# spaceandtimefdn/blitzar

Hardware: NVIDIA H100
Metric: MSM throughput (scalar*point terms/sec), ristretto255, n=2^20 per GPU (higher is better)
Workload: dtype u32 limbs (integer modular arithmetic)

## Files before the change

### blitzar_b200/csrc/curve.cuh

```cuda
#pragma once
#include "field.cuh"

namespace b200 {

enum CurveId : unsigned { kRistretto255 = 0, kBls12381 = 1, kBn254 = 2, kGrumpkin = 3 };

struct SeqExec {
  static constexpr int kLanes = 1;
  template <class F>
  static B200_HD void mul4(typename F::E& o0, typename F::E& o1, typename F::E& o2,
                           typename F::E& o3, const typename F::E& a0, const typename F::E& b0,
                           const typename F::E& a1, const typename F::E& b1,
                           const typename F::E& a2, const typename F::E& b2,
                           const typename F::E& a3, const typename F::E& b3) {
    F::mul(o0, a0, b0);
    F::mul(o1, a1, b1);
    F::mul(o2, a2, b2);
    F::mul(o3, a3, b3);
  }
  template <class F>
  static B200_HD void mul2(typename F::E& o0, typename F::E& o1, const typename F::E& a0,
                           const typename F::E& b0, const typename F::E& a1,
                           const typename F::E& b1) {
    F::mul(o0, a0, b0);
// ... 75 lines not shown
  struct Gen {
    fe YpX, YmX, Z2, T2d;
  };

  static B200_HD Point identity() {
    Point p;
    p.X = F::zero();
    p.Y = F::one();
    p.Z = F::one();
    p.T = F::zero();
    return p;
  }
  static B200_HD void neg(Point& r, const Point& a) {
    F::neg(r.X, a.X);
    r.Y = a.Y;
    r.Z = a.Z;
    F::neg(r.T, a.T);
  }
  template <class X = SeqExec> static B200_HD void add(Point& r, const Point& a, const Point& b) {
    fe A, B, C, D, E, Fv, G, H, t0, t1, t2, t3;
    F::sub(t0, a.Y, a.X);
    F::sub(t1, b.Y, b.X);
    F::add(t2, a.Y, a.X);
    F::add(t3, b.Y, b.X);
    X::template mul4<F>(A, B, C, D, t0, t1, t2, t3, a.T, b.T, a.Z, b.Z);
    F::mul(C, C, F::constant([](int i) { return F25_D2(i); }));
    F::dbl(D, D);
    F::sub(E, B, A);
    F::sub(Fv, D, C);
    F::add(G, D, C);
    F::add(H, B, A);
    Point o;
    X::template mul4<F>(o.X, o.Y, o.T, o.Z, E, Fv, G, H, E, H, Fv, G);
    r = o;
  }
  static B200_HD void point_to_gen(Gen& g, const Point& p) {
    F::add(g.YpX, p.Y, p.X);
    F::sub(g.YmX, p.Y, p.X);
    F::dbl(g.Z2, p.Z);
    F::mul(g.T2d, p.T, F::constant([](int i) { return F25_D2(i); }));
    F::canonical(g.YpX, g.YpX);
    F::canonical(g.YmX, g.YmX);
    F::canonical(g.Z2, g.Z2);
    F::canonical(g.T2d, g.T2d);
  }

  static B200_HD fe denominator(const Point& p) { return p.Z; }
  static B200_HD void normalized_gen(Gen& g, const Point& p, const fe& zi) {
    Point a;
    F::mul(a.X, p.X, zi);
    F::mul(a.Y, p.Y, zi);
    a.Z = F::one();
    F::mul(a.T, a.X, a.Y);
    point_to_gen(g, a);
  }
  static B200_HD void gen_to_point(Point& r, const Gen& g, bool negate) {
    fe x2, t2, nx, nt;
    F::sub(x2, g.YpX, g.YmX);
    F::add(r.Y, g.YpX, g.YmX);
    r.Z = g.Z2;
    F::mul(t2, g.T2d, F::constant([](int i) { return F25_INVD(i); }));
    F::neg(nx, x2);
    F::neg(nt, t2);
    F::select(r.X, x2, nx, negate);
    F::select(r.T, t2, nt, negate);
  }
  template <class X = SeqExec>
  static B200_HD void add_gen(Point& r, const Point& a, const Gen& g, bool negate,
                              bool unit_z = false) {
    fe A, B, C, D, E, Fv, G, H, t0, t1, qp, qm, qt, nt;
    F::select(qp, g.YpX, g.YmX, negate);
    F::select(qm, g.YmX, g.YpX, negate);
    F::neg(nt, g.T2d);
    F::select(qt, g.T2d, nt, negate);
    F::sub(t0, a.Y, a.X);
    F::add(t1, a.Y, a.X);
    if (unit_z) {
      F::mul(A, t0, qm);
      F::mul(B, t1, qp);
      F::mul(C, a.T, qt);
      F::dbl(D, a.Z);
    } else {
      X::template mul4<F>(A, B, C, D, t0, qm, t1, qp, a.T, qt, a.Z, g.Z2);
    }
    F::sub(E, B, A);
    F::sub(Fv, D, C);
    F::add(G, D, C);
    F::add(H, B, A);
    Point o;
    X::template mul4<F>(o.X, o.Y, o.T, o.Z, E, Fv, G, H, E, H, Fv, G);
    r = o;
  }
  template <class X = SeqExec> static B200_HD void dbl(Point& r, const Point& a) {
    fe A, B, C, E, Fv, G, H, t0, t1;
    F::add(t0, a.X, a.Y);
    X::template mul4<F>(A, B, C, t1, a.X, a.X, a.Y, a.Y, a.Z, a.Z, t0, t0);
    F::dbl(C, C);
    F::add(H, A, B);
    F::sub(E, H, t1);
    F::sub(G, A, B);
    F::add(Fv, C, G);
    Point o;
    X::template mul4<F>(o.X, o.Y, o.T, o.Z, E, Fv, G, H, E, H, Fv, G);
    r = o;
  }

  static B200_HD Gen load_unit_gen(const Gen* src) {
    Gen g;
    g.YpX = src->YpX;
    g.YmX = src->YmX;
    g.T2d = src->T2d;
    g.Z2 = F::zero();
    g.Z2.l[0] = 2;
    return g;
  }

  static B200_HD void load_point_abi(Point& p, const void* src) {
    const u64* s = (const u64*)src;
    F::from_radix51(p.X, s);
    F::from_radix51(p.Y, s + 5);
    F::from_radix51(p.Z, s + 10);
    F::from_radix51(p.T, s + 15);
  }
  static B200_HD fe load_abi_z(const void* src) {
    fe z;
    F::from_radix51(z, (const u64*)src + 10);
    return z;
  }
  static B200_HD void load_gen_abi(Gen& g, const void* src) {
    Point p;
    load_point_abi(p, src);
    point_to_gen(g, p);
  }
  static B200_HD void load_proj_abi(Gen& g, const void* src) { load_gen_abi(g, src); }
  static constexpr int kAbiCompactBytes = 120;
  static B200_HD void load_compact_abi(Gen& g, const void* src) {
    const u64* s = (const u64*)src;
    Point p;
    F::from_radix51(p.X, s);
    F::from_radix51(p.Y, s + 5);
    p.Z = F::one();
    F::from_radix51(p.T, s + 10);
    point_to_gen(g, p);
  }
  static B200_HD void store_compact_abi(void* dst, const Point& p, const fe& zi) {
    u64* d = (u64*)dst;
    fe x, y, t;
    F::mul(x, p.X, zi);
    F::mul(y, p.Y, zi);
    F::mul(t, x, y);
    F::to_radix51(d, x);
    F::to_radix51(d + 5, y);
    F::to_radix51(d + 10, t);
  }
  static B200_HD void store_proj_abi(void* dst, const Point& p) {
    u64* d = (u64*)dst;
    F::to_radix51(d, p.X);
    F::to_radix51(d + 5, p.Y);
    F::to_radix51(d + 10, p.Z);
    F::to_radix51(d + 15, p.T);
  }

  struct ScalarPow {
    static B200_HD void pow22523(fe& r, const fe& a) { F::pow22523(r, a); }
  };
  template <class Pow = ScalarPow> static B200_HD int sqrt_ratio_m1(fe& x, const fe& u, const fe& v) {
// ... 182 lines not shown
  }
  static B200_HD bool gen_is_identity(const Gen& g) { return F::is_zero(g.y) && F::is_zero(g.x); }
  static B200_HD Gen subgroup_generator() {
    Gen g;
#pragma unroll
    for (int i = 0; i < N; ++i) {
      g.x.l[i] = F::Params::gx(i);
      g.y.l[i] = F::Params::gy(i);
    }
    return g;
  }
  static B200_HD void neg(Point& r, const Point& a) {
    r.X = a.X;
    F::neg(r.Y, a.Y);
    r.Z = a.Z;
  }
  static B200_HD void mul_by_3b(fe& r, const fe& a) { CP::template mul_by_3b<F>(r, a); }

  template <class X>
  static B200_HD void finish_add(Point& r, const fe& t0, const fe& t1, const fe& t3, const fe& t4,
                                 const fe& y3, const fe& z3) {
    fe x3a, t2a, y3a, t1a, t0a, z3a;
    X::template mul4<F>(x3a, t2a, y3a, t1a, t4, y3, t3, t1, y3, t0, t1, z3);
    X::template mul2<F>(t0a, z3a, t0, t3, z3, t4);
    F::sub(r.X, t2a, x3a);
    F::add(r.Y, t1a, y3a);
    F::add(r.Z, z3a, t0a);
  }
  template <class X = SeqExec> static B200_HD void add(Point& r, const Point& p, const Point& q) {
    fe t0, t1, t2, t3, t4, m3, m4, m5, u0, u1, v0, v1, x3, y3, z3;
    F::add(t3, p.X, p.Y);
    F::add(t4, q.X, q.Y);
    F::add(u0, p.Y, p.Z);
    F::add(u1, q.Y, q.Z);
    F::add(v0, p.X, p.Z);
    F::add(v1, q.X, q.Z);
    X::template mul4<F>(t0, t1, t2, m3, p.X, q.X, p.Y, q.Y, p.Z, q.Z, t3, t4);
    X::template mul2<F>(m4, m5, u0, u1, v0, v1);
    F::add(t4, t0, t1);
    F::sub(t3, m3, t4);
    F::add(x3, t1, t2);
    F::sub(t4, m4, x3);
    F::add(y3, t0, t2);
    F::sub(y3, m5, y3);
    F::add(x3, t0, t0);
    F::add(t0, x3, t0);
    mul_by_3b(t2, t2);
    F::add(z3, t1, t2);
    F::sub(t1, t1, t2);
    mul_by_3b(y3, y3);
    Point o;
    finish_add<X>(o, t0, t1, t3, t4, y3, z3);
    r = o;
  }
  template <class X = SeqExec>
  static B200_HD void add_gen(Point& r, const Point& p, const Gen& g, bool negate,
                              bool  = false) {
    if (gen_is_identity(g)) {
      r = p;
      return;
    }
    fe qy, ny;
    F::neg(ny, g.y);
    F::select(qy, g.y, ny, negate);
    fe t0, t1, t2, t3, t4, m3, x3, y3, z3;
    F::add(t3, g.x, qy);
    F::add(t4, p.X, p.Y);
    X::template mul4<F>(t0, t1, m3, t2, p.X, g.x, p.Y, qy, t3, t4, qy, p.Z);
    F::mul(y3, g.x, p.Z);
    F::add(t4, t0, t1);
    F::sub(t3, m3, t4);
    F::add(t4, t2, p.Y);
    F::add(y3, y3, p.X);
    F::add(x3, t0, t0);
    F::add(t0, x3, t0);
    mul_by_3b(t2, p.Z);
    F::add(z3, t1, t2);
    F::sub(t1, t1, t2);
    mul_by_3b(y3, y3);
    Point o;
    finish_add<X>(o, t0, t1, t3, t4, y3, z3);
    r = o;
  }
  static B200_HD fe denominator(const Point& p) { return F::is_zero(p.Z) ? F::one() : p.Z; }
  static B200_HD void normalized_gen(Gen& g, const Point& p, const fe& zi) {
    if (F::is_zero(p.Z)) {
      g.x = F::zero();
      g.y = F::zero();
      return;
    }
    F::mul(g.x, p.X, zi);
    F::mul(g.y, p.Y, zi);
  }
  static B200_HD void gen_to_point(Point& r, const Gen& g, bool negate) {
    if (gen_is_identity(g)) {
      r = identity();
      return;
    }
    fe ny;
    F::neg(ny, g.y);
    r.X = g.x;
    F::select(r.Y, g.y, ny, negate);
    r.Z = F::one();
  }
  template <class X = SeqExec> static B200_HD void dbl(Point& r, const Point& p) {
    fe t0, t1, t2, txy, x3, y3, z3, xa, xb;
    X::template mul4<F>(t0, t1, t2, txy, p.Y, p.Y, p.Y, p.Z, p.Z, p.Z, p.X, p.Y);
    F::add(z3, t0, t0);
    F::add(z3, z3, z3);
    F::add(z3, z3, z3);
    mul_by_3b(t2, t2);
    F::add(y3, t0, t2);
    fe t22, t23;
    F::add(t22, t2, t2);
    F::add(t23, t22, t2);
    F::sub(t0, t0, t23);
    Point o;
    X::template mul4<F>(xa, o.Z, y3, xb, t2, z3, t1, z3, t0, y3, t0, txy);
    F::add(o.Y, xa, y3);
    F::add(o.X, xb, xb);
    r = o;
  }

  static B200_HD void load_gen_abi(Gen& g, const void* src) {
    const unsigned char* s = (const unsigned char*)src;
    if (s[8 * N]) {
      g.x = F::zero();
      g.y = F::zero();
      return;
    }
    F::load(g.x, s);
    F::load(g.y, s + 4 * N);
  }
  static constexpr int kAbiCompactBytes = 8 * N;
  static B200_HD void load_compact_abi(Gen& g, const void* src) {
    const u32* s = (const u32*)src;
    if ((s[N - 1] & s[N - 2]) == 0xffffffffu) {
      g.x = F::zero();
      g.y = F::zero();
      return;
    }
    F::load(g.x, s);
    F::load(g.y, s + N);
  }
  static B200_HD void store_compact_abi(void* dst, const Point& p, const fe& zi) {
    u32* d = (u32*)dst;
    fe x, y;
    if (F::is_zero(p.Z)) {
      x = F::zero();
      x.l[N - 2] = x.l[N - 1] = 0xffffffffu;
      y = F::one();
    } else {
      F::mul(x, p.X, zi);
      F::mul(y, p.Y, zi);
    }
    F::store(d, x);
    F::store(d + N, y);
  }
  static B200_HD void load_proj_abi(Gen& g, const void* src) {
    const unsigned char* s = (const unsigned char*)src;
    fe X, Y, Z, zi;
    F::load(X, s);
    F::load(Y, s + 4 * N);
    F::load(Z, s + 8 * N);
    if (F::is_zero(Z)) {
      g.x = F::zero();
// ... 114 lines not shown
```

### blitzar_b200/csrc/msm.cuh

```cuda
#pragma once
#include <algorithm>
#include <vector>

#include "batch_affine.cuh"
#include "curve.cuh"
#include "engine_api.cuh"
#include "lanefield.cuh"

namespace b200 {

struct ColumnDesc {
  const unsigned char* base;
  u64 row_stride;
  u32 bit_offset;
  u32 bit_width;
  u32 n;
  u32 is_signed;
  u32 first_window;
  u32 num_windows;
  u32 table_n;
  u32 gen_base;
};
B200_HD u32 bucket_windows(const ColumnDesc& col) { return col.table_n ? (col.num_windows ? 1u : 0u) : col.num_windows; }

// ... 475 lines not shown
      entries[(u64)lo + i] = sorted[i];
  }
};

inline u32 binned_sort_shift(u64 nkeys) {
  u32 shift = 0;
  while ((nkeys + (1ull << shift) - 1) >> shift > kMicroBins)
    ++shift;
  return shift;
}

inline void binned_sort(stream_t s, const ColumnDesc* d_cols, const u64* d_col_start, u32 ncols,
                        u32 c, u32 nbuckets, u64 total_terms, u64 max_entries, u32 max_windows,
                        u64 nkeys, u64* entries, u32* counts, u32* d_m) {
  const u32 shift = binned_sort_shift(nkeys);
  const u32 nmicro = (u32)((nkeys + (1ull << shift) - 1) >> shift);
  const u32 span_micro = std::max(1u, kBinSpan >> shift);
  u32* ws = (u32*)dev_alloc((5ull * nmicro + 3) * sizeof(u32), s);
  u32 *micro_counts = ws, *bin_of = ws + nmicro, *bin_cursor = ws + 2ull * nmicro,
      *bin_start = ws + 3ull * nmicro, *bin_micro = ws + 4ull * nmicro + 1,
      *nbins = ws + 5ull * nmicro + 2;
  u64* tmp = (u64*)dev_alloc(std::max<u64>(max_entries, 1) * sizeof(u64), s);
  dev_zero(micro_counts, nmicro * sizeof(u32), s);
  const u64 count_tile = 4096;
  launch_blocks(MicroCountBody{d_cols, d_col_start, ncols, c, nbuckets, total_terms,
                               (u32)count_tile, shift, nmicro, micro_counts},
                (total_terms + count_tile - 1) / count_tile, nmicro * sizeof(u32), s);
  launch_blocks(PlanBinsBody{micro_counts, nmicro, span_micro, nkeys, bin_of, bin_start, bin_micro,
                             bin_cursor, nbins, counts, d_m},
                1, nmicro * sizeof(u32), s);
  const size_t scatter_smem = 220 * 1024;
  const size_t bin_bytes = (2ull * nmicro + 2) * sizeof(u32);
  const u64 stage_entries = (scatter_smem - bin_bytes) / sizeof(u64);
  const u64 scatter_tile = std::max<u64>(1, stage_entries / max_windows);
  launch_blocks(CoarseScatterBody{d_cols, d_col_start, ncols, c, nbuckets, total_terms,
                                  (u32)scatter_tile, shift, nmicro, bin_of, nbins, bin_cursor, tmp},
                (total_terms + scatter_tile - 1) / scatter_tile, scatter_smem, s);
  launch_blocks(BinSortBody{tmp, bin_start, bin_micro, nbins, shift, nkeys, entries, counts}, nmicro,
                BinSortBody::kSmem, s);
  dev_free(tmp, s);
  dev_free(ws, s);
}
#endif

template <class C> struct FillIdentityBody {
  static constexpr int kBlock = 256;
  static constexpr u32 kChunks = sizeof(typename C::Point) / 16;
  static_assert(sizeof(typename C::Point) % 16 == 0, "points are made of 16-byte aligned fields");
  uint4* p;
  B200_HD void operator()(u64 t) const {
    const typename C::Point id = C::identity();
    const u32 k = (u32)(t % kChunks);
    uint4 v = ((const uint4*)&id)[0];
#pragma unroll
    for (u32 j = 1; j < kChunks; ++j)
      if (j == k)
        v = ((const uint4*)&id)[j];
    p[t] = v;
  }
};
template <class C> inline void fill_identity(stream_t s, typename C::Point* p, u64 n) {
  launch(FillIdentityBody<C>{(uint4*)p}, n * FillIdentityBody<C>::kChunks, s);
}

template <class C> struct MergeBucketsBody {
  static constexpr int kBlock = 128;
  const u32* bucket_end;
  const u32* bucket_begin;
  const typename C::Point* scratch;
  typename C::Point* buckets;
  B200_HD void operator()(u64 k) const {
    const u32 lo = bucket_begin ? bucket_begin[k] : (k ? bucket_end[k - 1] : 0u);
    if (bucket_end[k] == lo)
      return;
    typename C::Point b = buckets[k];
    C::add(b, b, scratch[k]);
    buckets[k] = b;
  }
};

template <class C, bool kGather, class X = SeqExec, bool kUniform = false, bool kUnitZ = false>
struct AccumulateBody {
  static constexpr int kBlock = 128;
  static constexpr int kMinBlocks = !kGather ? 1 : (C::F::N > 8 ? 2 : 3);
  typedef typename C::Point Point;
  typedef typename C::Gen Gen;
  const u32* keys;
  const u64* entries;
  const Gen* gens;
  const Point* pieces;
  const u32* m_ptr;
  u32 K;
  u32 final_level;
  Point* buckets;
  u32* out_keys;
  Point* out_pieces;
  u32* out_m_ptr;
  const u32* unit_veto;

  B200_HD void put_bucket(u32 key, const Point& acc, bool writer) const {
    if (writer)
      buckets[key] = acc;
  }
  B200_HD u32 key_at(u64 i) const { return kGather ? (u32)(entries[i] >> 32) : keys[i]; }
  B200_HD void fetch(Point& acc, u64 i, bool first) const {
    if (kGather) {
      u32 e = (u32)entries[i];
      if (first)
        C::gen_to_point(acc, gens[e >> 1], e & 1u);
      else
        C::template add_gen<X>(acc, acc, gens[e >> 1], e & 1u);
    } else {
      if (first)
        acc = pieces[i];
      else
        C::template add<X>(acc, acc, pieces[i]);
    }
  }
  template <bool kUnit> B200_HD Gen load_gen(u32 idx) const {
    if constexpr (kUnit)
      return C::load_unit_gen(gens + idx);
    else
      return gens[idx];
  }
  template <bool kUnit>
  B200_HD void gather_walk(u64 t, u64 b, u64 e, bool writer, u32& cur, Point& acc,
                           bool& first_seg) const {
    u64 ent = entries[b];
    Gen g = load_gen<kUnit>((u32)ent >> 1);
    cur = (u32)(ent >> 32);
    struct {
      Point p;
      B200_HD void start(const Gen& g, bool negate) { C::gen_to_point(p, g, negate); }
      B200_HD void add(const Gen& g, bool negate) {
        C::template add_gen<X>(p, p, g, negate, kUnit);
      }
      B200_HD void get(Point& out) const { out = p; }
    } ga;
    for (u64 i = b; i < e; ++i) {
      u64 ent_n = ent;
      Gen g_n = g;
      if (i + 1 < e) {
        ent_n = entries[i + 1];
        g_n = load_gen<kUnit>((u32)ent_n >> 1);
      }
      const u32 k = (u32)(ent >> 32);
      const bool negate = ((u32)ent & 1u) != 0;
      if (kUniform) {
        if (i == b) {
          ga.p = C::identity();
        } else if (k != cur) {
          ga.get(acc);
          if (final_level || !first_seg) {
            put_bucket(cur, acc, writer);
          } else if (writer) {
            out_keys[2 * t] = cur;
            out_pieces[2 * t] = acc;
          }
          first_seg = false;
          cur = k;
          ga.p = C::identity();
        }
        ga.add(g, negate);
      } else if (i == b) {
        ga.start(g, negate);
      } else if (k == cur) {
        ga.add(g, negate);
      } else {
        ga.get(acc);
        if (final_level || !first_seg) {
          put_bucket(cur, acc, writer);
        } else if (writer) {
          out_keys[2 * t] = cur;
          out_pieces[2 * t] = acc;
        }
        first_seg = false;
        cur = k;
        ga.start(g, negate);
      }
      ent = ent_n;
      g = g_n;
    }
    ga.get(acc);
  }
  B200_HD void operator()(u64 tid) const {
    const u64 t = tid / X::kLanes;
    const bool writer = (tid % X::kLanes) == 0;
    const u64 M = *m_ptr;
    const u64 T = (M + K - 1) / K;
    if (tid == 0 && out_m_ptr)
      *out_m_ptr = final_level ? 0u : (u32)(2 * T);
    u64 b = t * K;
    if (b >= M)
      return;
    u64 e = b + K < M ? b + K : M;
    u32 cur;
    Point acc;
    bool first_seg = true;
    if (kGather) {
      if (kUnitZ && unit_veto && *unit_veto)
        gather_walk<false>(t, b, e, writer, cur, acc, first_seg);
      else
        gather_walk<kUnitZ>(t, b, e, writer, cur, acc, first_seg);
    } else {
      cur = key_at(b);
      fetch(acc, b, true);
      for (u64 i = b + 1; i < e; ++i) {
        u32 k = key_at(i);
        if (k == cur) {
          fetch(acc, i, false);
        } else {
          if (final_level || !first_seg) {
            put_bucket(cur, acc, writer);
          } else if (writer) {
            out_keys[2 * t] = cur;
            out_pieces[2 * t] = acc;
          }
          first_seg = false;
          cur = k;
          fetch(acc, i, true);
        }
      }
    }
    if (final_level) {
      put_bucket(cur, acc, writer);
      return;
    }
    if (!writer)
      return;
    if (first_seg) {
      out_keys[2 * t] = cur;
      out_pieces[2 * t] = acc;
      out_keys[2 * t + 1] = cur;
      out_pieces[2 * t + 1] = C::identity();
    } else {
      out_keys[2 * t + 1] = cur;
      out_pieces[2 * t + 1] = acc;
    }
  }
};

struct WindowUsedBody {
  static constexpr int kBlock = 64;
  const u32* bucket_end;
  u32 nbuckets;
  u32* window_used;
  B200_HD void operator()(u64 w) const {
    u32 lo = w ? bucket_end[w * nbuckets - 1] : 0u;
    u32 hi = bucket_end[(w + 1) * nbuckets - 1];
    if (hi != lo)
      window_used[w] = 1u;
  }
};

struct WindowUsedFromCountsBody {
  static constexpr int kBlock = 128;
  const u32* counts;
  u64 nkeys;
  u32 nbuckets;
  u32* window_used;
  B200_HD void operator()(u64 t) const {
    const u64 b = t * 256, e = b + 256 < nkeys ? b + 256 : nkeys;
    for (u64 k = b; k < e; ++k)
      if (counts[k])
        window_used[k / nbuckets] = 1u;
  }
};

template <class C, class Ex = SeqExec> struct ReduceBody {
  static constexpr int kBlock = 64;
  typedef typename C::Point Point;
  const Point* X;
  const Point* Cin;
  u32 m_in, g, log2g;
  Point* Xout;
  Point* Cout;
  const u32* window_used;
  u32 nbuckets;
  B200_HD void operator()(u64 tid) const {
    const u64 t = tid / Ex::kLanes;
    const bool writer = (tid % Ex::kLanes) == 0;
    const u32 m_out = m_in / g;
    const u32 w = (u32)(t / m_out), k = (u32)(t % m_out);
    if (window_used[w] == 0) {
      if (writer) {
        Xout[t] = C::identity();
// ... 600 lines not shown
    }
    const bool window_major = opt.scatter_window_major && r.max_windows > 1;
    launch(ScatterBody{r.d_cols, r.d_col_start, ncols, c, nbuckets, out.counts, out.entries,
                       window_major ? total_terms : 0},
           window_major ? total_terms * r.max_windows : total_terms, s);
  }
  if (L)
    launch(FillPadsBody{out.starts, out.counts, out.entries}, nkeys, s);
  else
    launch(WindowUsedBody{out.counts, nbuckets, window_used}, plan.total_windows, s);
  return out;
}

inline unsigned sort_selftest(stream_t s, std::vector<ColumnDesc> cols, u32 c) {
  MsmOptions opt;
  opt.window_bits = c;
  const MsmPlan plan = msm_make_plan(std::move(cols), opt, 160);
  const StagedRange r(s, plan, 0, plan.max_n);
  if (r.total_terms == 0)
    return ~0u;
  const u64 nkeys = plan.nkeys, M = r.max_entries;
  DevBuf<u32> window_used(plan.total_windows, s);
  opt.sort_path = 0;
  const SortedLayout a = sort_entries(s, plan, r, 0, opt, window_used.p);
  opt.sort_path = 2;
  const SortedLayout b = sort_entries(s, plan, r, 0, opt, window_used.p);
  std::vector<u32> ca(nkeys + 1), cb(nkeys + 1), m(1);
  std::vector<u64> ea(M), eb(M);
  copy_d2h(ca.data(), a.counts, (nkeys + 1) * sizeof(u32), s);
  copy_d2h(cb.data(), b.counts, (nkeys + 1) * sizeof(u32), s);
  copy_d2h(m.data(), b.d_m, sizeof(u32), s);
  copy_d2h(ea.data(), a.entries, M * sizeof(u64), s);
  copy_d2h(eb.data(), b.entries, M * sizeof(u64), s);
  stream_sync(s);
  for (void* p : {(void*)a.entries, (void*)a.counts, (void*)a.d_m, (void*)b.entries, (void*)b.counts,
                  (void*)b.d_m, (void*)r.d_cols})
    dev_free(p, s);
  if (!b.binned)
    return ~0u;
  unsigned bad = m[0] == ca[nkeys] ? 0u : 1u;
  for (u64 k = 0; k < nkeys; ++k) {
    const u32 lo = k ? ca[k - 1] : 0u, hi = ca[k];
    if (cb[k] != hi || hi < lo || hi > M) {
      ++bad;
      continue;
    }
    std::sort(ea.begin() + lo, ea.begin() + hi);
    std::sort(eb.begin() + lo, eb.begin() + hi);
    if (!std::equal(ea.begin() + lo, ea.begin() + hi, eb.begin() + lo))
      ++bad;
  }
  return bad;
}

struct RangeHook {
  virtual void before_range(u64 begin, u64 end) = 0;
  virtual void before_accumulate() {}
  virtual ~RangeHook() {}
};

template <class C>
stream_t chunk_walk(stream_t s, stream_t tail, WalkInput<C> walk, u32* d_m, bool unit,
                    const u32* unit_veto, typename C::Point* target, const MsmOptions& opt,
                    std::vector<void*>& to_free) {
  typedef typename C::Point Point;
  u32 K = opt.chunk1 ? std::max(opt.chunk1, 4u) : (walk.m_max >= (1ull << 23) ? 64u : 32u);
  const u32 chunkn = std::max(opt.chunkn, 4u);
  const u32* lvl_keys = nullptr;
  const Point* lvl_pieces = nullptr;
  stream_t cs = s;
  for (int level = 0;; ++level) {
    const bool final_level = walk.m_max <= K;
    u64 T = (walk.m_max + K - 1) / K;
    u32* out_keys = final_level ? nullptr : (u32*)dev_alloc(2 * T * sizeof(u32), cs);
    Point* out_pieces = final_level ? nullptr : (Point*)dev_alloc(2 * T * sizeof(Point), cs);
    to_free.insert(to_free.end(), {out_keys, out_pieces});
    u32* out_m = d_m + 1 + (level % 8);
    if (level == 0) {
      const bool uniform =
          opt.uniform_add == 2 ? C::kCurveId == kRistretto255 : opt.uniform_add != 0;
      constexpr bool kEd = C::kCurveId == kRistretto255;
      const bool unit_path = kEd && unit;
      if (uniform && unit_path)
        launch(AccumulateBody<C, true, SeqExec, true, kEd>{nullptr, walk.entries, walk.gens, nullptr,
                                                            walk.m_ptr, K, final_level, target,
                                                            out_keys, out_pieces, out_m, unit_veto},
               T, s);
      else if (uniform)
        launch(AccumulateBody<C, true, SeqExec, true>{nullptr, walk.entries, walk.gens, nullptr,
                                                      walk.m_ptr, K, final_level, target, out_keys,
                                                      out_pieces, out_m, nullptr},
               T, s);
      else if (unit_path)
        launch(AccumulateBody<C, true, SeqExec, false, kEd>{nullptr, walk.entries, walk.gens, nullptr,
                                                             walk.m_ptr, K, final_level, target,
                                                             out_keys, out_pieces, out_m, unit_veto},
               T, s);
      else
        launch(AccumulateBody<C, true>{nullptr, walk.entries, walk.gens, nullptr, walk.m_ptr, K,
                                       final_level, target, out_keys, out_pieces, out_m, nullptr},
               T, s);
      KernelTimer::get().end(s);
      if (tail != s)
        stream_follow(tail, s);
      cs = tail;
    } else if (T <= opt.quad_threshold) {
      launch(AccumulateBody<C, false, QuadExec>{lvl_keys, nullptr, nullptr, lvl_pieces, walk.m_ptr,
                                                K, final_level, target, out_keys, out_pieces, out_m,
                                                nullptr},
             T * QuadExec::kLanes, cs);
    } else {
      launch(AccumulateBody<C, false>{lvl_keys, nullptr, nullptr, lvl_pieces, walk.m_ptr, K,
                                      final_level, target, out_keys, out_pieces, out_m, nullptr},
             T, cs);
    }
    if (final_level)
      break;
    lvl_keys = out_keys;
    lvl_pieces = out_pieces;
    walk.m_ptr = out_m;
    walk.m_max = 2 * T;
    K = chunkn;
  }
  return cs;
}

template <class C>
void msm_accumulate_range(stream_t s, const MsmPlan& plan, const typename C::Gen* gens, u64 begin,
                          u64 end, bool add_into, typename C::Point* d_buckets,
                          u32* d_window_used, const MsmOptions& opt, stream_t tail,
                          RangeHook* hook = nullptr) {
  const StagedRange r(s, plan, begin, end);
  if (r.total_terms == 0)
    return;
  gens += begin;
  StageRange nvtx_sort("msm: digit count + scan + scatter");
  const u64 max_entries = r.max_entries, nkeys = plan.nkeys;
  u32 L = 0;
  if constexpr (C::kBatchAffine) {
    const double mean = (double)max_entries / (double)nkeys;
    if (opt.pair_levels >= 0)
      L = (u32)opt.pair_levels;
    else if (max_entries >= (1ull << 23))
      while (L < 6 && (double)(32u << L) <= mean)
        ++L;
    while (L > 0 && max_entries + nkeys * ((1ull << L) - 1) >= (1ull << 32) - (1ull << L))
      --L;
  }
  const SortedLayout sorted = sort_entries(s, plan, r, L, opt, d_window_used);
  B200_LOG(3, "range [%llu, %llu): %llu terms, %llu entries max, c=%u, %llu keys, pair levels %u",
           (unsigned long long)begin, (unsigned long long)end, (unsigned long long)r.total_terms,
           (unsigned long long)max_entries, plan.c, (unsigned long long)nkeys, L);
  WalkInput<C> walk{gens, sorted.entries, sorted.d_m, max_entries};
  std::vector<void*> to_free;
  if (hook)
    hook->before_accumulate();
  KernelTimer::get().begin(s);
  StageRange nvtx_acc("msm: bucket accumulation");
  if constexpr (C::kBatchAffine) {
    if (L) {
      walk = run_pair_levels<C>(s, L, sorted.entries, gens, sorted.d_m, sorted.slots_max,
                                opt.pair_batch);
      to_free = {(void*)walk.gens, (void*)walk.entries};
    }
  }
  typedef typename C::Point Point;
  Point* target = add_into ? (Point*)dev_alloc(nkeys * sizeof(Point), s) : d_buckets;
  const bool unit = walk.gens == gens && opt.gens_normalized;
  const stream_t cs =
      chunk_walk<C>(s, tail, walk, sorted.d_m, unit, opt.unit_veto, target, opt, to_free);
  if (add_into) {
    launch(MergeBucketsBody<C>{sorted.counts, sorted.starts, target, d_buckets}, nkeys, cs);
    dev_free(target, cs);
  }
  to_free.insert(to_free.end(), {sorted.d_m, sorted.counts, sorted.starts});
  for (void* ptr : to_free)
    dev_free(ptr, cs);
  dev_free(sorted.entries, s);
  dev_free((void*)r.d_cols, s);
}

template <class C>
void msm_finish(stream_t s, const MsmPlan& plan, const typename C::Point* d_buckets,
                const u32* d_window_used, typename C::Point* out, const MsmOptions& opt) {
// ... 112 lines not shown
```

### blitzar_b200/csrc/runtime.cuh

```cuda
#pragma once
#include <cstdio>
#include <cstdlib>
#include <cstring>
#include <atomic>
#include <cctype>
#include <string>
#include <utility>
#include <vector>

#include "field.cuh"

#ifndef B200_EMULATE
#include <cuda_runtime.h>
#include <nvtx3/nvToolsExt.h>
#endif

namespace b200 {

[[noreturn]] inline void die(const char* what, const char* file, int line) {
  std::fprintf(stderr, "blitzar_b200: fatal: %s (%s:%d)\n", what, file, line);
  std::abort();
}
#define B200_REQUIRE(cond, msg)                                                                    \
  do {                                                                                             \
    if (!(cond))                                                                                   \
      ::b200::die(msg, __FILE__, __LINE__);                                                        \
  } while (0)

inline int log_level() {
  static const int level = [] {
    const char* env = std::getenv("BLITZAR_LOG_LEVEL");
    if (!env)
      return 0;
    std::string s(env);
    for (auto& ch : s)
      ch = (char)std::tolower((unsigned char)ch);
    if (s == "warn")
      return 1;
    if (s == "info")
      return 2;
    if (s == "debug" || s == "trace")
      return 3;
    return 0;
  }();
  return level;
}
#define B200_LOG(level, ...)                                                                       \
  do {                                                                                             \
    if (::b200::log_level() >= (level)) {                                                          \
      std::fprintf(stderr, "[blitzar_b200] " __VA_ARGS__);                                         \
      std::fputc('\n', stderr);                                                                    \
    }                                                                                              \
  } while (0)

struct StageRange {
#ifndef B200_EMULATE
  explicit StageRange(const char* name) { nvtxRangePushA(name); }
  ~StageRange() { nvtxRangePop(); }
#else
  explicit StageRange(const char*) {}
#endif
  StageRange(const StageRange&) = delete;
  StageRange& operator=(const StageRange&) = delete;
};

#ifndef B200_EMULATE
#define B200_CUDA(call)                                                                            \
  do {                                                                                             \
    cudaError_t e_ = (call);                                                                       \
    if (e_ != cudaSuccess)                                                                         \
      ::b200::die(cudaGetErrorString(e_), __FILE__, __LINE__);                                     \
  } while (0)

typedef cudaStream_t stream_t;

template <class Body, class = void> struct MinBlocks {
  static constexpr int value = 1;
};
template <class Body> struct MinBlocks<Body, decltype((void)Body::kMinBlocks)> {
  static constexpr int value = Body::kMinBlocks;
};
template <class Body>
__global__ void __launch_bounds__(Body::kBlock, MinBlocks<Body>::value) k_run(Body body, u64 n) {
  u64 tid = (u64)blockIdx.x * blockDim.x + threadIdx.x;
  if (tid < n)
    body(tid);
}

struct LaunchCounter {
  static std::atomic<unsigned long long>& value() {
    static std::atomic<unsigned long long> v{0};
    return v;
  }
};

template <class Body> inline void launch(const Body& body, u64 n, stream_t s) {
  if (n == 0)
    return;
  u64 blocks = (n + Body::kBlock - 1) / Body::kBlock;
  B200_REQUIRE(blocks < (1ull << 31), "grid too large");
  k_run<Body><<<(unsigned)blocks, Body::kBlock, 0, s>>>(body, n);
  B200_CUDA(cudaGetLastError());
  ++LaunchCounter::value();
}
template <class Body> __global__ void __launch_bounds__(Body::kBlock) k_block(Body body) {
  extern __shared__ __align__(16) unsigned char smem[];
  body.run(blockIdx.x, smem);
}
template <class Body>
inline void launch_blocks(const Body& body, u64 blocks, size_t smem_bytes, stream_t s) {
  if (blocks == 0)
    return;
  B200_REQUIRE(blocks < (1ull << 31), "grid too large");
  static thread_local size_t raised = 48 * 1024;
  if (smem_bytes > raised) {
    B200_CUDA(cudaFuncSetAttribute(k_block<Body>, cudaFuncAttributeMaxDynamicSharedMemorySize,
                                   (int)smem_bytes));
    raised = smem_bytes;
  }
  k_block<Body><<<(unsigned)blocks, Body::kBlock, smem_bytes, s>>>(body);
  B200_CUDA(cudaGetLastError());
  ++LaunchCounter::value();
}
inline void* dev_alloc(size_t bytes, stream_t s) {
  void* p = nullptr;
  B200_CUDA(cudaMallocAsync(&p, bytes ? bytes : 16, s));
  return p;
}
inline void dev_free(void* p, stream_t s) {
  if (p)
    B200_CUDA(cudaFreeAsync(p, s));
}
inline void dev_zero(void* p, size_t bytes, stream_t s) { B200_CUDA(cudaMemsetAsync(p, 0, bytes, s)); }
inline void copy_h2d(void* d, const void* h, size_t bytes, stream_t s) {
  if (bytes)
    B200_CUDA(cudaMemcpyAsync(d, h, bytes, cudaMemcpyHostToDevice, s));
}
inline void copy_d2h(void* h, const void* d, size_t bytes, stream_t s) {
  if (bytes)
    B200_CUDA(cudaMemcpyAsync(h, d, bytes, cudaMemcpyDeviceToHost, s));
}
inline void copy_d2d(void* d, const void* s_, size_t bytes, stream_t s) {
  if (bytes)
    B200_CUDA(cudaMemcpyAsync(d, s_, bytes, cudaMemcpyDeviceToDevice, s));
}
inline void stream_sync(stream_t s) { B200_CUDA(cudaStreamSynchronize(s)); }
inline void stream_follow(stream_t later, stream_t earlier) {
  static thread_local cudaEvent_t ring[64];
  static thread_local unsigned next = 0;
  cudaEvent_t& e = ring[next++ % 64];
  if (!e)
    B200_CUDA(cudaEventCreateWithFlags(&e, cudaEventDisableTiming));
  B200_CUDA(cudaEventRecord(e, earlier));
  B200_CUDA(cudaStreamWaitEvent(later, e, 0));
}

inline stream_t aux_stream() {
  static thread_local cudaStream_t s = nullptr;
  if (!s)
    B200_CUDA(cudaStreamCreateWithFlags(&s, cudaStreamNonBlocking));
  return s;
}

struct StagingRing {
  static constexpr size_t kSlotBytes = 65536, kSlots = 128;
  unsigned char* base = nullptr;
  cudaEvent_t done[kSlots];
  size_t next = 0;
  static StagingRing& get() {
    static thread_local StagingRing r;
    return r;
  }
  void* stage(stream_t s, const void* host, size_t bytes) {
    void* d = dev_alloc(bytes, s);
    if (bytes > kSlotBytes) {
      copy_h2d(d, host, bytes, s);
      stream_sync(s);
      return d;
    }
    if (!base) {
      B200_CUDA(cudaHostAlloc((void**)&base, kSlotBytes * kSlots, cudaHostAllocDefault));
      for (auto& e : done) {
        B200_CUDA(cudaEventCreateWithFlags(&e, cudaEventDisableTiming));
      }
    }
    size_t slot = next++ % kSlots;
    B200_CUDA(cudaEventSynchronize(done[slot]));
    std::memcpy(base + slot * kSlotBytes, host, bytes);
    B200_CUDA(cudaMemcpyAsync(d, base + slot * kSlotBytes, bytes, cudaMemcpyHostToDevice, s));
    B200_CUDA(cudaEventRecord(done[slot], s));
    return d;
  }
};
inline void* stage_to_device(stream_t s, const void* host, size_t bytes) {
  return StagingRing::get().stage(s, host, bytes);
}

struct KernelTimer {
  bool enabled = false;
  std::vector<std::pair<cudaEvent_t, cudaEvent_t>> spans;
  static KernelTimer& get() {
    static thread_local KernelTimer t;
    return t;
  }
  void begin(stream_t s) {
    if (!enabled)
      return;
    cudaEvent_t a, b;
    B200_CUDA(cudaEventCreate(&a));
    B200_CUDA(cudaEventCreate(&b));
    B200_CUDA(cudaEventRecord(a, s));
    spans.emplace_back(a, b);
  }
  void end(stream_t s) {
    if (!enabled)
      return;
    B200_CUDA(cudaEventRecord(spans.back().second, s));
  }
  void read(float* total_ms, unsigned* count) {
    float tot = 0;
    for (auto& sp : spans) {
      float ms = 0;
      B200_CUDA(cudaEventSynchronize(sp.second));
      B200_CUDA(cudaEventElapsedTime(&ms, sp.first, sp.second));
      tot += ms;
      B200_CUDA(cudaEventDestroy(sp.first));
      B200_CUDA(cudaEventDestroy(sp.second));
    }
    *total_ms = tot;
    *count = (unsigned)spans.size();
    spans.clear();
  }
};
template <class T> B200_HD T atomic_add(T* p, T v) {
#ifdef __CUDA_ARCH__
  return atomicAdd(p, v);
#else
  T old = *p;
  *p = old + v;
  return old;
#endif
}
#define B200_ATOMIC_ADD(ptr, v) ::b200::atomic_add((ptr), (v))
#else
typedef int stream_t;
struct LaunchCounter {
  static unsigned long long& value() {
    static unsigned long long v = 0;
    return v;
  }
};
template <class Body> inline void launch(const Body& body, u64 n, stream_t) {
  for (u64 t = 0; t < n; ++t)
    body(t);
  ++LaunchCounter::value();
}
inline void* dev_alloc(size_t bytes, stream_t) { return std::malloc(bytes ? bytes : 16); }
inline void dev_free(void* p, stream_t) { std::free(p); }
inline void dev_zero(void* p, size_t bytes, stream_t) { std::memset(p, 0, bytes); }
inline void copy_h2d(void* d, const void* h, size_t bytes, stream_t) { std::memcpy(d, h, bytes); }
inline void copy_d2h(void* h, const void* d, size_t bytes, stream_t) { std::memcpy(h, d, bytes); }
inline void copy_d2d(void* d, const void* s_, size_t bytes, stream_t) { std::memcpy(d, s_, bytes); }
inline void stream_sync(stream_t) {}
inline void stream_follow(stream_t, stream_t) {}
inline stream_t aux_stream() { return 0; }
inline void* stage_to_device(stream_t s, const void* host, size_t bytes) {
  void* d = dev_alloc(bytes, s);
  std::memcpy(d, host, bytes);
  return d;
}
struct KernelTimer {
  static KernelTimer& get() {
    static KernelTimer t;
    return t;
  }
  void begin(stream_t) {}
  void end(stream_t) {}
};
template <class T> inline T emul_atomic_add(T* p, T v) {
  T old = *p;
  *p = old + v;
  return old;
}
#define B200_ATOMIC_ADD(ptr, v) ::b200::emul_atomic_add((ptr), (v))
#endif

}
```

Before: 335.2 million.

## Prefetch gathered generators into shared memory ring via cp.async in accumulate

The gather-accumulate walk now stages upcoming generator points into a per-thread two-slot shared-memory ring using cp.async, instead of prefetching the next generator into registers. The ristretto addition reads operands straight from shared memory through a new pointer-based add_gen_at. This is meant to cut register pressure and hide global gather latency. The minimum blocks per SM for ristretto255 is raised from 3 to 4. A new smem launch path is added, at the cost of per-block shared memory, which could limit occupancy, and an async wait on every step.

```diff
diff --git a/blitzar_b200/csrc/curve.cuh b/blitzar_b200/csrc/curve.cuh
--- a/blitzar_b200/csrc/curve.cuh
+++ b/blitzar_b200/csrc/curve.cuh
@@ -181,6 +181,36 @@
       F::dbl(D, a.Z);
     } else {
       X::template mul4<F>(A, B, C, D, t0, qm, t1, qp, a.T, qt, a.Z, g.Z2);
+    }
+    F::sub(E, B, A);
+    F::sub(Fv, D, C);
+    F::add(G, D, C);
+    F::add(H, B, A);
+    Point o;
+    X::template mul4<F>(o.X, o.Y, o.T, o.Z, E, Fv, G, H, E, H, Fv, G);
+    r = o;
+  }
+  template <class X = SeqExec>
+  static B200_HD void add_gen_at(Point& r, const Point& a, const Gen* g, bool negate,
+                                 bool unit_z = false) {
+    fe A, B, C, D, E, Fv, G, H, t0, t1, qt, nt;
+    const fe* qm = negate ? &g->YpX : &g->YmX;
+    const fe* qp = negate ? &g->YmX : &g->YpX;
+    F::sub(t0, a.Y, a.X);
+    F::add(t1, a.Y, a.X);
+    if (unit_z) {
+      F::mul(A, t0, *qm);
+      F::mul(B, t1, *qp);
+      qt = g->T2d;
+      F::neg(nt, qt);
+      F::select(qt, qt, nt, negate);
+      F::mul(C, a.T, qt);
+      F::dbl(D, a.Z);
+    } else {
+      qt = g->T2d;
+      F::neg(nt, qt);
+      F::select(qt, qt, nt, negate);
+      X::template mul4<F>(A, B, C, D, t0, *qm, t1, *qp, a.T, qt, a.Z, g->Z2);
     }
     F::sub(E, B, A);
     F::sub(Fv, D, C);
@@ -529,6 +559,12 @@
     finish_add<X>(o, t0, t1, t3, t4, y3, z3);
     r = o;
   }
+  template <class X = SeqExec>
+  static B200_HD void add_gen_at(Point& r, const Point& p, const Gen* g, bool negate,
+                                 bool unit_z = false) {
+    const Gen q = *g;
+    add_gen<X>(r, p, q, negate, unit_z);
+  }
   static B200_HD fe denominator(const Point& p) { return F::is_zero(p.Z) ? F::one() : p.Z; }
   static B200_HD void normalized_gen(Gen& g, const Point& p, const fe& zi) {
     if (F::is_zero(p.Z)) {
diff --git a/blitzar_b200/csrc/msm.cuh b/blitzar_b200/csrc/msm.cuh
--- a/blitzar_b200/csrc/msm.cuh
+++ b/blitzar_b200/csrc/msm.cuh
@@ -581,9 +581,17 @@
 template <class C, bool kGather, class X = SeqExec, bool kUniform = false, bool kUnitZ = false>
 struct AccumulateBody {
   static constexpr int kBlock = 128;
-  static constexpr int kMinBlocks = !kGather ? 1 : (C::F::N > 8 ? 2 : 3);
+  static constexpr int kMinBlocks =
+      !kGather ? 1 : (C::F::N > 8 ? 2 : (C::kCurveId == kRistretto255 ? 4 : 3));
   typedef typename C::Point Point;
   typedef typename C::Gen Gen;
+  static constexpr int kRing = 2;
+  static constexpr u32 kGenChunks = sizeof(Gen) / 16;
+  static constexpr u32 kThreadBytes = (kRing * kGenChunks + 1) * 16;
+  static_assert(sizeof(Gen) % 16 == 0 && kGenChunks % 2 == 0, "odd 16-byte thread stride");
+  static constexpr size_t smem_bytes() {
+    return kGather ? (size_t)kBlock * (kThreadBytes + kRing * sizeof(u64)) : 0;
+  }
   const u32* keys;
   const u64* entries;
   const Gen* gens;
@@ -616,33 +624,62 @@
         C::template add<X>(acc, acc, pieces[i]);
     }
   }
-  template <bool kUnit> B200_HD Gen load_gen(u32 idx) const {
-    if constexpr (kUnit)
-      return C::load_unit_gen(gens + idx);
-    else
-      return gens[idx];
+  template <bool kUnit> static B200_HD bool chunk_needed(u32 j) {
+    if constexpr (kUnit) {
+      constexpr u32 z = offsetof(Gen, Z2) / 16, zn = sizeof(typename C::fe) / 16;
+      return j < z || j >= z + zn;
+    } else {
+      return true;
+    }
   }
   template <bool kUnit>
   B200_HD void gather_walk(u64 t, u64 b, u64 e, bool writer, u32& cur, Point& acc,
-                           bool& first_seg) const {
-    u64 ent = entries[b];
-    Gen g = load_gen<kUnit>((u32)ent >> 1);
-    cur = (u32)(ent >> 32);
+                           bool& first_seg, unsigned char* smem, u32 lane) const {
+    constexpr int P = kRing - 1;
+    Gen* ring = (Gen*)(smem + lane * kThreadBytes);
+    u64* ring_ent = (u64*)(smem + kBlock * kThreadBytes) + lane;
+    auto issue = [&](u64 w, int s) {
+      const uint4* src = (const uint4*)(gens + ((u32)w >> 1));
+      uint4* dst = (uint4*)(ring + s);
+#pragma unroll
+      for (u32 j = 0; j < kGenChunks; ++j)
+        if (chunk_needed<kUnit>(j))
+          copy16_async(dst + j, src + j);
+      ring_ent[s * kBlock] = w;
+    };
+#pragma unroll
+    for (int s = 0; s < P; ++s) {
+      if (b + s < e)
+        issue(entries[b + s], s);
+      async_commit();
+    }
+    u64 w_ahead = b + P < e ? entries[b + P] : 0;
+    cur = (u32)(entries[b] >> 32);
     struct {
       Point p;
-      B200_HD void start(const Gen& g, bool negate) { C::gen_to_point(p, g, negate); }
-      B200_HD void add(const Gen& g, bool negate) {
-        C::template add_gen<X>(p, p, g, negate, kUnit);
+      B200_HD void start(const Gen* g, bool negate) {
+        if constexpr (kUnit)
+          C::gen_to_point(p, C::load_unit_gen(g), negate);
+        else
+          C::gen_to_point(p, *g, negate);
+      }
+      B200_HD void add(const Gen* g, bool negate) {
+        C::template add_gen_at<X>(p, p, g, negate, kUnit);
       }
       B200_HD void get(Point& out) const { out = p; }
     } ga;
+    int s_use = 0;
     for (u64 i = b; i < e; ++i) {
-      u64 ent_n = ent;
-      Gen g_n = g;
-      if (i + 1 < e) {
-        ent_n = entries[i + 1];
-        g_n = load_gen<kUnit>((u32)ent_n >> 1);
+      if (i + P < e) {
+        issue(w_ahead, s_use == 0 ? P : s_use - 1);
+        if (i + P + 1 < e)
+          w_ahead = entries[i + P + 1];
       }
+      async_commit();
+      async_wait<P>();
+      const u64 ent = ring_ent[s_use * kBlock];
+      const Gen* g = ring + s_use;
+      s_use = s_use == P ? 0 : s_use + 1;
       const u32 k = (u32)(ent >> 32);
       const bool negate = ((u32)ent & 1u) != 0;
       if (kUniform) {
@@ -677,12 +714,10 @@
         cur = k;
         ga.start(g, negate);
       }
-      ent = ent_n;
-      g = g_n;
     }
     ga.get(acc);
   }
-  B200_HD void operator()(u64 tid) const {
+  B200_HD void operator()(u64 tid, unsigned char* smem = nullptr) const {
     const u64 t = tid / X::kLanes;
     const bool writer = (tid % X::kLanes) == 0;
     const u64 M = *m_ptr;
@@ -697,10 +732,11 @@
     Point acc;
     bool first_seg = true;
     if (kGather) {
+      const u32 lane = (u32)(tid % kBlock);
       if (kUnitZ && unit_veto && *unit_veto)
-        gather_walk<false>(t, b, e, writer, cur, acc, first_seg);
+        gather_walk<false>(t, b, e, writer, cur, acc, first_seg, smem, lane);
       else
-        gather_walk<kUnitZ>(t, b, e, writer, cur, acc, first_seg);
+        gather_walk<kUnitZ>(t, b, e, writer, cur, acc, first_seg, smem, lane);
     } else {
       cur = key_at(b);
       fetch(acc, b, true);
@@ -1467,24 +1503,26 @@
       constexpr bool kEd = C::kCurveId == kRistretto255;
       const bool unit_path = kEd && unit;
       if (uniform && unit_path)
-        launch(AccumulateBody<C, true, SeqExec, true, kEd>{nullptr, walk.entries, walk.gens, nullptr,
-                                                            walk.m_ptr, K, final_level, target,
-                                                            out_keys, out_pieces, out_m, unit_veto},
-               T, s);
+        launch_smem(AccumulateBody<C, true, SeqExec, true, kEd>{nullptr, walk.entries, walk.gens,
+                                                                 nullptr, walk.m_ptr, K, final_level,
+                                                                 target, out_keys, out_pieces, out_m,
+                                                                 unit_veto},
+                    T, s);
       else if (uniform)
-        launch(AccumulateBody<C, true, SeqExec, true>{nullptr, walk.entries, walk.gens, nullptr,
-                                                      walk.m_ptr, K, final_level, target, out_keys,
-                                                      out_pieces, out_m, nullptr},
-               T, s);
+        launch_smem(AccumulateBody<C, true, SeqExec, true>{nullptr, walk.entries, walk.gens, nullptr,
+                                                           walk.m_ptr, K, final_level, target,
+                                                           out_keys, out_pieces, out_m, nullptr},
+                    T, s);
       else if (unit_path)
-        launch(AccumulateBody<C, true, SeqExec, false, kEd>{nullptr, walk.entries, walk.gens, nullptr,
-                                                             walk.m_ptr, K, final_level, target,
-                                                             out_keys, out_pieces, out_m, unit_veto},
-               T, s);
+        launch_smem(AccumulateBody<C, true, SeqExec, false, kEd>{nullptr, walk.entries, walk.gens,
+                                                                  nullptr, walk.m_ptr, K, final_level,
+                                                                  target, out_keys, out_pieces, out_m,
+                                                                  unit_veto},
+                    T, s);
       else
-        launch(AccumulateBody<C, true>{nullptr, walk.entries, walk.gens, nullptr, walk.m_ptr, K,
-                                       final_level, target, out_keys, out_pieces, out_m, nullptr},
-               T, s);
+        launch_smem(AccumulateBody<C, true>{nullptr, walk.entries, walk.gens, nullptr, walk.m_ptr, K,
+                                            final_level, target, out_keys, out_pieces, out_m, nullptr},
+                    T, s);
       KernelTimer::get().end(s);
       if (tail != s)
         stream_follow(tail, s);
diff --git a/blitzar_b200/csrc/runtime.cuh b/blitzar_b200/csrc/runtime.cuh
--- a/blitzar_b200/csrc/runtime.cuh
+++ b/blitzar_b200/csrc/runtime.cuh
@@ -100,6 +100,29 @@
   u64 blocks = (n + Body::kBlock - 1) / Body::kBlock;
   B200_REQUIRE(blocks < (1ull << 31), "grid too large");
   k_run<Body><<<(unsigned)blocks, Body::kBlock, 0, s>>>(body, n);
+  B200_CUDA(cudaGetLastError());
+  ++LaunchCounter::value();
+}
+template <class Body>
+__global__ void __launch_bounds__(Body::kBlock, MinBlocks<Body>::value) k_run_smem(Body body, u64 n) {
+  extern __shared__ __align__(16) unsigned char smem[];
+  u64 tid = (u64)blockIdx.x * blockDim.x + threadIdx.x;
+  if (tid < n)
+    body(tid, smem);
+}
+template <class Body> inline void launch_smem(const Body& body, u64 n, stream_t s) {
+  if (n == 0)
+    return;
+  u64 blocks = (n + Body::kBlock - 1) / Body::kBlock;
+  B200_REQUIRE(blocks < (1ull << 31), "grid too large");
+  const size_t smem_bytes = Body::smem_bytes();
+  static thread_local size_t raised = 48 * 1024;
+  if (smem_bytes > raised) {
+    B200_CUDA(cudaFuncSetAttribute(k_run_smem<Body>, cudaFuncAttributeMaxDynamicSharedMemorySize,
+                                   (int)smem_bytes));
+    raised = smem_bytes;
+  }
+  k_run_smem<Body><<<(unsigned)blocks, Body::kBlock, smem_bytes, s>>>(body, n);
   B200_CUDA(cudaGetLastError());
   ++LaunchCounter::value();
 }
@@ -255,6 +278,13 @@
     body(t);
   ++LaunchCounter::value();
 }
+template <class Body> inline void launch_smem(const Body& body, u64 n, stream_t) {
+  std::vector<unsigned char> smem(Body::smem_bytes() + 16);
+  unsigned char* base = (unsigned char*)(((uintptr_t)smem.data() + 15) & ~(uintptr_t)15);
+  for (u64 t = 0; t < n; ++t)
+    body(t, base);
+  ++LaunchCounter::value();
+}
 inline void* dev_alloc(size_t bytes, stream_t) { return std::malloc(bytes ? bytes : 16); }
 inline void dev_free(void* p, stream_t) { std::free(p); }
 inline void dev_zero(void* p, size_t bytes, stream_t) { std::memset(p, 0, bytes); }
@@ -285,4 +315,24 @@
 #define B200_ATOMIC_ADD(ptr, v) ::b200::emul_atomic_add((ptr), (v))
 #endif
 
-}
+B200_HD void copy16_async(void* smem_dst, const void* gmem_src) {
+#ifdef __CUDA_ARCH__
+  asm volatile("cp.async.cg.shared.global [%0], [%1], 16;" ::"r"((u32)__cvta_generic_to_shared(smem_dst)),
+               "l"(__cvta_generic_to_global(gmem_src))
+               : "memory");
+#else
+  std::memcpy(smem_dst, gmem_src, 16);
+#endif
+}
+B200_HD void async_commit() {
+#ifdef __CUDA_ARCH__
+  asm volatile("cp.async.commit_group;" ::: "memory");
+#endif
+}
+template <int N> B200_HD void async_wait() {
+#ifdef __CUDA_ARCH__
+  asm volatile("cp.async.wait_group %0;" ::"n"(N) : "memory");
+#endif
+}
+
+}
```

New measurement: 338.4 million (median of 6 runs). About the same (+0.9%).
